# xdu-Liu-learn/Video-desensitization

Hardware: AMD Instinct MI355X
Metric: end-to-end detect+blur FPS on 1920x1080 frames (higher is better)
Workload: dtype fp32; 1 GPU; RetinaFace-R50+FPN+SSH + YOLOv8n plates detect + mosaic write-back, 64 frames of 1920x1080 per step over 1 GPU(s) (batches of 64 per GPU); global_batch=64, frame=1920x1080, net_input=640x640, parallelism=frame-sharded x1, plates=True, batches_in_flight=1

## Files before the change

video-desensitization_amd/csrc/conv_x6.hip:

```cpp
#include "vd_kernel.h"
#include "conv_x6.h"
#include <algorithm>
#include <type_traits>
#include <cmath>
#include <cstring>

namespace {

template <int BM, int BN, int NT, int NST, int TERMS, int MF, bool TR = false, bool PF = false>
__global__ __launch_bounds__(NT, NT == 256 && BM == 256 ? 1 : 2) void conv_x6_kernel(ConvArgs a) {
    static_assert(MF == 16 || (MF == 32 && TERMS == 2), "32x32x16 form: fp16 pairs only");
    static_assert(!TR || (MF == 16 && TERMS == 2), "TR tiles: fp16 pairs on 16x16x32");
    using S = X6Shape<BM, BN, NT, NST, TERMS, MF>;
    constexpr int NA = 2;
    constexpr int STAGE = S::STAGE, PL_A = S::PL_A, PL_B = S::PL_B, TM = S::TM, TN = S::TN, WAVES = S::WAVES;
    constexpr int AROWS = S::AROWS, AIT = S::AITEMS;
    extern __shared__ __attribute__((aligned(16))) char smem[];
    const int tid = threadIdx.x, lane = tid & 63, wid = tid >> 6;
    const int wm = wid / S::WAVES_N, wn = wid % S::WAVES_N;

    const int nwg = gridDim.x, bid = blockIdx.x;
    const int q8 = nwg >> 3, r8 = nwg & 7, xcd = bid & 7;
    const int wg = (xcd < r8 ? xcd * (q8 + 1) : r8 * (q8 + 1) + (xcd - r8) * q8) + (bid >> 3);
    const int tn = wg % a.ntiles_n, tm = wg / a.ntiles_n;
// ... 405 lines not shown
    hipError_t err = hipSuccess;
    if (vd_launch_x6_stream(a, TERMS, s, &err)) return err;
    if constexpr (TERMS == 2) {
        if (a.tune->x6_gemm1x1 && x6_tr_ok(a)) return launch_tr(a, s);
    }
    const int bn = a.cout <= 32 ? 32 : (a.cout <= 64 ? 64 : 128);
    const long big_tiles = (long)((a.M + 255) / 256) * ((a.cout + bn - 1) / bn);
    const int small_k = a.tune->x6_small_k, small_tiles = a.tune->x6_small_tiles, small_k2 = a.tune->x6_small_k2;
    const bool force_small = small_k >= (1 << 30);
    const bool small = force_small || (bn <= 64 && (a.kpad <= (TERMS == 2 ? small_k2 : small_k) ||
                                                    big_tiles < small_tiles));
    if constexpr (TERMS == 2) {
        if (bn <= 64 && a.tune->x6_halo_narrow && vd_x6_halo_ok(a)) return vd_launch_x6_halo(a, bn, s);
    }
    if (small) {
        if constexpr (TERMS == 2) {
            if (bn == 32 && a.x_exact) return launch_x6<128, 32, 256, 1, 1>(a, s);
            if (bn == 64 && a.x_exact) return launch_x6<128, 64, 256, 1, 1>(a, s);
        }
        if (bn == 32) return launch_x6<128, 32, 256, 1, TERMS>(a, s);
        if (bn == 64) return launch_x6<128, 64, 256, 1, TERMS>(a, s);
        return launch_x6<128, 128, 256, 1, TERMS>(a, s);
    }
    if (bn == 32) return launch_x6<256, 32, 512, 2, TERMS>(a, s);
    if (bn == 64) return launch_x6<256, 64, 512, 2, TERMS>(a, s);
    if constexpr (TERMS == 2) {
        if (a.tune->x6_mid && a.kh == 1 && a.kw == 1 && a.kpad <= a.tune->x6_mid && a.cout == 128)
            return launch_x6<128, 128, 256, 2, TERMS>(a, s);
    }
    if constexpr (TERMS == 2) {
        const long t256 = (long)((a.M + 255) / 256) * (a.cout / 256);
        if (a.tune->x6_bn256 && a.cout % 256 == 0 && t256 >= 192) {
            if (vd_x6_halo_ok(a)) return vd_launch_x6_halo(a, 256, s);
            if (a.tune->x6_mf32) return launch_x6<256, 256, 512, 2, TERMS, 32>(a, s);
            return launch_x6<256, 256, 512, 2, TERMS>(a, s);
        }
        if (a.tune->x6_bn256 && a.cout == 192 && (a.M + 255) / 256 >= 192) {
            if (vd_x6_halo_ok(a)) return vd_launch_x6_halo(a, 192, s);
            return launch_x6<256, 192, 512, 2, TERMS>(a, s);
        }
        if (vd_x6_halo_ok(a)) return vd_launch_x6_halo(a, 128, s);
        if (a.tune->x6_mf32) return launch_x6<256, 128, 512, 2, TERMS, 32>(a, s);
    }
    return launch_x6<256, 128, 512, 2, TERMS>(a, s);
}

hipError_t vd_launch_conv_x6(const ConvArgs& a0, hipStream_t s) {
    if (!a0.tune) return hipErrorInvalidValue;
    ConvArgs a = a0;
    a.one = a.tune->x6_one != 0;
    a.halo_dma = a.tune->x6_halo_dma & 3;
    a.gemm_1b = a.tune->x6_gemm_uni == 2;
    a.halo_1b = a.tune->x6_halo_1b != 0;
    a.dbg = a.tune->x6_dbg & 0x3d;
    if (a.grp_co) {
        if (a.grp_co != 64 || a.f32_split != 2 || !a.wx3 || !vd_x6_halo_ok(a) || (a.ymax && a.B > kAmaxFrames))
            return hipErrorInvalidValue;
        a.scale = a.scale_x;
        return vd_launch_x6_halo(a, 64, s);
    }
    if (a.x2) {
        if (!vd_conv1x1_x6_dual_ok(a) || (a.ymax && a.B > kAmaxFrames)) return hipErrorInvalidValue;
        return vd_launch_x6_dual(a, s);
    }
    if (a.f32_split == 2) {
        if (!a.scale_x || (a.ymax && a.B > kAmaxFrames)) return hipErrorInvalidValue;
        return launch_terms<2>(a, s);
    }
    ConvArgs b = a;
    b.xmax = nullptr;
    return launch_terms<3>(b, s);
}

static inline unsigned f2u(float f) { unsigned u; std::memcpy(&u, &f, 4); return u; }
static inline float u2f(unsigned u) { float f; std::memcpy(&f, &u, 4); return f; }

void vd_pack_x6(const float* w, int npad, int kpad, uint16_t* out) {
    const int nk = kpad / KT;
    for (int n = 0; n < npad; ++n)
        for (int t = 0; t < nk; ++t)
            for (int k = 0; k < KT; ++k) {
                const float x = w[(size_t)n * kpad + t * KT + k];
                const unsigned u = f2u(x);
                const float r1 = x - u2f(u & 0xFFFF0000u);
                const unsigned v = f2u(r1);
                const float r2 = r1 - u2f(v & 0xFFFF0000u);
                uint16_t* o = out + (((size_t)n * nk + t) * 3) * KT + k;
                o[0] = (uint16_t)(u >> 16);
                o[KT] = (uint16_t)(v >> 16);
                o[2 * KT] = (uint16_t)(f2u(r2) >> 16);
            }
}

void vd_pack_x3h(const float* w, int npad, int kpad, uint16_t* out, float* row_inv) {
    const int nk = kpad / KT;
    for (int n = 0; n < npad; ++n) {
        float m = 0.f;
        for (int k = 0; k < kpad; ++k) m = std::max(m, std::fabs(w[(size_t)n * kpad + k]));
        int e = 0;
        if (m > 0.f) {
            (void)std::frexp(m, &e);
            e = std::min(100, std::max(-100, 15 - e));
        }
        row_inv[n] = std::ldexp(1.f, -e);
        for (int t = 0; t < nk; ++t)
            for (int k = 0; k < KT; ++k) {
// ... 10 lines not shown
```

video-desensitization_amd/csrc/conv_x6_halo.hip:

```cpp
#include "vd_kernel.h"
#include "conv_x6.h"
#include <algorithm>

namespace {

__device__ __forceinline__ int swzh(int row, int chunk) { return row * 64 + ((chunk ^ (((row >> 2) & 1) << 1)) << 4); }

__host__ __device__ __forceinline__ constexpr int s2_tap(int j) {
    return j == 0 ? 8 : j == 1 ? 6 : j == 2 ? 2 : j == 3 ? 0 : j == 4 ? 7 : j == 5 ? 1 : j == 6 ? 5 : j == 7 ? 3 : 4;
}
__host__ __device__ __forceinline__ constexpr bool s2_last(int j) { return j == 3 || j == 5 || j == 7 || j == 8; }

template <int BN, int NSB, bool TR = false, bool S2 = false, bool PF = false>
__global__ __launch_bounds__(512, BN <= 64 ? 4 : 2) void conv_x6_halo_kernel(ConvArgs a) {
    using S = X6Shape<256, BN, 512, 2, 2>;
    constexpr int BM = 256, NT = 512, TM = S::TM, TN = S::TN, WAVES = S::WAVES, PL_B = S::PL_B;
    constexpr int QI = 4;
    extern __shared__ __attribute__((aligned(16))) char smem[];
    const int tid = threadIdx.x, lane = tid & 63, wid = tid >> 6;
    const int wm = wid / S::WAVES_N, wn = wid % S::WAVES_N;
    const int nwg = gridDim.x, bid = blockIdx.x;
    const int q8 = nwg >> 3, r8 = nwg & 7, xcd = bid & 7;
    const int wg = (xcd < r8 ? xcd * (q8 + 1) : r8 * (q8 + 1) + (xcd - r8) * q8) + (bid >> 3);
    const int tn = wg % a.ntiles_n, tm = wg / a.ntiles_n;
    const int m0 = tm * BM, n0 = tn * BN;
    static_assert(!S2 || (NSB == 3 && S::NDMA % WAVES == 0), "stride-2 halo: three B stages, whole DMA rounds");
    const int W = a.yw, H = a.yh, HW = H * W;
    const int HR = S2 ? BM + W + 1 : BM + 2 * W + 2, HP = HR + 1;
    const int PL_H = HP * 64;
    char* Ah = smem + NSB * 2 * PL_B;
    const int CH = a.cin_pad / 32, nsteps = 9 * CH, nk = a.kpad / KT;
    const int nhalo = S2 ? 4 * CH : CH;

    const long xbytes = (long)a.B * a.xh * a.xw * a.ldx * 4;
    const __amdgpu_buffer_rsrc_t rsrc_x = __builtin_amdgcn_make_buffer_rsrc((void*)a.x, 0, (int)xbytes, 0x00020000);
    int hoff[QI];
    unsigned hexp = 0;
    unsigned hodd = 0;
    const int xg = a.grp_co ? (n0 / a.grp_co) * a.grp_ci : 0;
#pragma unroll
    for (int q = 0; q < QI; ++q) {
        const int it = tid + NT * q, hr = it >> 2, pr = it & 3;
        const int pix = m0 - W - 1 + hr;
        const bool ok = hr < HR && pix >= 0 && pix < a.M;
        if constexpr (S2) {
            const int b = pix / HW, rem = pix - b * HW, yo = rem / W, xo = rem - yo * W;
            hoff[q] = ok ? ((b * a.xh + 2 * yo) * a.xw + 2 * xo) * a.ldx + a.xcoff + xg + pr * 8 : -1;
            hodd |= (unsigned)((2 * yo + 1 < a.xh ? 1 : 0) | (2 * xo + 1 < a.xw ? 2 : 0)) << (2 * q);
        } else {
            hoff[q] = ok ? pix * a.ldx + a.xcoff + xg + pr * 8 : -1;
        }
        hexp |= (unsigned)((ok ? act_scale_exp(a, pix / HW) : 0) & 0xff) << (8 * q);
    }
    u32x4 hx[QI][2];
    auto load_halo = [&](int h) {
        const int c = S2 ? h >> 2 : h, ph = S2 ? 3 - (h & 3) : 0, py = ph >> 1, px = ph & 1;
        const int dph = (py * a.xw + px) * a.ldx;
        const unsigned need = (unsigned)(py | (px << 1));
#pragma unroll
        for (int q = 0; q < QI; ++q) {
            const bool v = hoff[q] >= 0 && (!S2 || ((hodd >> (2 * q)) & need) == need);
            const unsigned off = v ? (unsigned)(hoff[q] + dph + c * KT) * 4u : 0x80000000u;
            hx[q][0] = __builtin_bit_cast(u32x4, __builtin_amdgcn_raw_buffer_load_b128(rsrc_x, (int)off, 0, 0));
            hx[q][1] = __builtin_bit_cast(u32x4, __builtin_amdgcn_raw_buffer_load_b128(rsrc_x, (int)off, 16, 0));
        }
    };
    auto store_halo = [&]() {
#pragma unroll
        for (int q = 0; q < QI; ++q) {
            const int it = tid + NT * q, hr = it >> 2, pr = it & 3;
            if (hr < HR) {
                float e[8];
#pragma unroll
                for (int j = 0; j < 4; ++j) {
                    e[j] = __uint_as_float(hx[q][0][j]);
                    e[4 + j] = __uint_as_float(hx[q][1][j]);
                }
                u32x4 o[3];
                const int ex = (int)(signed char)((hexp >> (8 * q)) & 0xff);
                split_pack<2>(e, __builtin_ldexpf(1.f, ex), o);
                *(u32x4*)(Ah + swzh(hr, pr)) = o[0];
                *(u32x4*)(Ah + PL_H + swzh(hr, pr)) = o[1];
            }
        }
    };

    constexpr int RB = BN / 16, NDMA = S::NDMA;
    const int my_dma = NDMA / WAVES + (wid < NDMA % WAVES ? 1 : 0);
    const __amdgpu_buffer_rsrc_t rsrc_w = __builtin_amdgcn_make_buffer_rsrc((void*)a.w, 0, 0x7fffffff, 0x00020000);
    auto dma_piece = [&](int s, int st, int q) {
        const int c = s / 9, j = s - 9 * c, kt = (S2 ? s2_tap(j) : j) * CH + c;
        char* Bs = smem + st * 2 * PL_B;
        const int jd = wid + WAVES * q;
        if (jd < NDMA) {
            const int p = jd / RB, r0 = (jd % RB) * 16;
            const int row = r0 + (lane >> 2), slot = lane & 3;
            const int chunk = slot ^ (((row >> 3) & 1) * 3);
            const int wrow = TR ? x6_tr_row(row) : row;
            const unsigned off = (unsigned)((((long)(n0 + wrow) * nk + kt) * 2 + p) * 64 + chunk * 16);
            __builtin_amdgcn_raw_ptr_buffer_load_lds(rsrc_w, (lds_void_t*)(Bs + p * PL_B + r0 * 64), 16, off, 0,
                                                     0, 0);
        }
    };
    auto dma_b = [&](int s, int st) {
#pragma unroll
        for (int q = 0; q < (NDMA + WAVES - 1) / WAVES; ++q) dma_piece(s, st, q);
    };
    constexpr int MYD = S::NDMA % WAVES == 0 ? S::NDMA / WAVES : 0;
    const int hdma = MYD ? a.halo_dma & 3 : 0;
    const int hdbg = (a.dbg >> 2) & 15;

    int arow[TM], aflg[TM];
#pragma unroll
    for (int i = 0; i < TM; ++i) {
        const int r = wm * S::WTM + i * 16 + (lane & 15), m = m0 + r;
        const int rem = m % HW, y = rem / W, x = rem - y * W;
        arow[i] = r + W + 1;
        aflg[i] = (y > 0 ? 1 : 0) | (y < H - 1 ? 2 : 0) | (x > 0 ? 4 : 0) | (x < W - 1 ? 8 : 0) | (m < a.M ? 16 : 0);
    }

    using AccT = f32x4_t;
    AccT acc[TM][TN];
#pragma unroll
    for (int i = 0; i < TM; ++i)
#pragma unroll
        for (int j = 0; j < TN; ++j) acc[i][j] = AccT{};
    const int amax_off = std::max(NSB * 2 * PL_B + 2 * PL_H, S::EPR * S::EPLD * 4);
    if (a.ymax)
        for (int f = tid; f < a.B; f += NT) ((unsigned*)(smem + amax_off))[f] = 0u;

    auto compute = [&](int st, int dy, int dx, int dstep) {
        const char* Bs = smem + st * 2 * PL_B;
        const int ch = lane >> 4;
        const int need = S2 ? (dy < 0 ? 1 : 0) | (dx < 0 ? 4 : 0) | 16
                            : (dy < 0 ? 1 : 0) | (dy > 0 ? 2 : 0) | (dx < 0 ? 4 : 0) | (dx > 0 ? 8 : 0) | 16;
        const int shift = S2 ? (dy < 0 ? -W : 0) + (dx < 0 ? -1 : 0) : dy * W + dx;
        if constexpr (TN < TM) {
            u32x4 bf[TN][3];
#pragma unroll
            for (int j = 0; j < TN; ++j) {
                bf[j][0] = *(const u32x4*)(Bs + swz64(wn * S::WTN + j * 16 + (lane & 15), ch));
                bf[j][1] = *(const u32x4*)(Bs + PL_B + swz64(wn * S::WTN + j * 16 + (lane & 15), ch));
            }
#pragma unroll
            for (int i = 0; i < TM; ++i) {
                const int hr = (aflg[i] & need) == need ? arow[i] + shift : HR;
                const int o = swzh(hr, ch);
                u32x4 af[3];
                af[0] = *(const u32x4*)(Ah + o);
                af[1] = *(const u32x4*)(Ah + PL_H + o);
#pragma unroll
                for (int j = 0; j < TN; ++j) {
                    if constexpr (TR) acc[i][j] = mfma_pair_tr(af, bf[j], acc[i][j]);
                    else acc[i][j] = mfma_pair(af, bf[j], acc[i][j]);
                }
            }
        } else if constexpr (PF) {
            u32x4 af[TM][3], bq[2][3];
#pragma unroll
            for (int i = 0; i < TM; ++i) {
                const int hr = (aflg[i] & need) == need ? arow[i] + shift : HR;
                const int o = swzh(hr, ch);
                af[i][0] = *(const u32x4*)(Ah + o);
                af[i][1] = *(const u32x4*)(Ah + PL_H + o);
            }
            bq[0][0] = *(const u32x4*)(Bs + swz64(wn * S::WTN + (lane & 15), ch));
            bq[0][1] = *(const u32x4*)(Bs + PL_B + swz64(wn * S::WTN + (lane & 15), ch));
            __builtin_amdgcn_sched_group_barrier(0x0100, 2 * TM + 2, 0);
#pragma unroll
            for (int j = 0; j < TN; ++j) {
                if (j + 1 < TN) {
                    bq[(j + 1) & 1][0] = *(const u32x4*)(Bs + swz64(wn * S::WTN + (j + 1) * 16 + (lane & 15), ch));
                    bq[(j + 1) & 1][1] = *(const u32x4*)(Bs + PL_B + swz64(wn * S::WTN + (j + 1) * 16 + (lane & 15), ch));
                    __builtin_amdgcn_sched_group_barrier(0x0100, 2, 0);
                }
#pragma unroll
                for (int i = 0; i < TM; ++i) {
                    if constexpr (TR) acc[i][j] = mfma_pair_tr(af[i], bq[j & 1], acc[i][j]);
                    else acc[i][j] = mfma_pair(af[i], bq[j & 1], acc[i][j]);
                }
                __builtin_amdgcn_sched_group_barrier(0x0008, 3 * TM, 0);
                if constexpr (MYD > 0 && TN % MYD == 0) {
                    if (dstep >= 0 && j % (TN / MYD) == 0) dma_piece(dstep, dstep % NSB, j / (TN / MYD));
                }
            }
        } else {
            u32x4 af[TM][3];
#pragma unroll
            for (int i = 0; i < TM; ++i) {
                const int hr = (aflg[i] & need) == need ? arow[i] + shift : HR;
                const int o = swzh(hr, ch);
                af[i][0] = *(const u32x4*)(Ah + o);
                af[i][1] = *(const u32x4*)(Ah + PL_H + o);
            }
#pragma unroll
            for (int j = 0; j < TN; ++j) {
                u32x4 bf[3];
                bf[0] = *(const u32x4*)(Bs + swz64(wn * S::WTN + j * 16 + (lane & 15), ch));
                bf[1] = *(const u32x4*)(Bs + PL_B + swz64(wn * S::WTN + j * 16 + (lane & 15), ch));
#pragma unroll
                for (int i = 0; i < TM; ++i) {
                    if constexpr (TR) acc[i][j] = mfma_pair_tr(af[i], bf, acc[i][j]);
                    else acc[i][j] = mfma_pair(af[i], bf, acc[i][j]);
                }
                if constexpr (MYD > 0 && TN % MYD == 0) {
                    if (dstep >= 0 && j % (TN / MYD) == 0) dma_piece(dstep, dstep % NSB, j / (TN / MYD));
                }
            }
        }
    };

    load_halo(0);
    store_halo();
    if (tid < 8) *(u32x4*)(Ah + (tid >> 2) * PL_H + swzh(HR, tid & 3)) = u32x4{0u, 0u, 0u, 0u};
    dma_b(0, 0);
    const bool one_bar = NSB == 2 && MYD > 0 && a.halo_1b;
    if (nsteps > 1 && !one_bar) dma_b(1, 1);
    if (nhalo > 1) load_halo(1);
    if constexpr (NSB == 3 && S::NDMA % WAVES == 0) {
        int hcur = 0;
        for (int s = 0; s < nsteps; ++s) {
            const int tap = s % 9;
            const bool ended = s >= 1 && (S2 ? s2_last(tap == 0 ? 8 : tap - 1) : tap == 0);
            const bool halo_prev = ended ? hcur + 1 < nhalo : (s <= 1 && nhalo > 1);
            if (halo_prev) {
                if (s + 1 < nsteps) wait_vm_k<MYD + 2 * QI>();
                else wait_vm_k<2 * QI>();
            } else {
                if (s + 1 < nsteps) wait_vm_k<MYD>();
                else wait_vm_k<0>();
            }
            asm volatile("s_waitcnt lgkmcnt(0)" ::: "memory");
            if (!(hdbg & 8)) __builtin_amdgcn_s_barrier();
            asm volatile("" ::: "memory");
            const bool rehalo = (S2 ? s2_last(tap) : tap == 8) && hcur + 1 < nhalo;
            const bool dnext = !rehalo && s + 2 < nsteps && !(hdbg & 1);
            const int hd = (TN % (MYD ? MYD : 1) == 0 && TN >= TM) ? hdma : (hdma ? 1 : 0);
            if (dnext && hd == 0) dma_b(s + 2, (s + 2) % 3);
            const int wt = S2 ? s2_tap(tap) : tap;
            const int dy = wt / 3 - 1, dx = wt - (wt / 3) * 3 - 1;
            compute(s % 3, dy, dx, dnext && hd == 2 ? s + 2 : -1);
            if (dnext && hd == 1) dma_b(s + 2, (s + 2) % 3);
            if (rehalo) {
                asm volatile("s_waitcnt lgkmcnt(0)" ::: "memory");
                if (!(hdbg & 8)) __builtin_amdgcn_s_barrier();
                asm volatile("" ::: "memory");
                if (!(hdbg & 2)) store_halo();
                ++hcur;
                if (hcur + 1 < nhalo && !(hdbg & 2)) load_halo(hcur + 1);
                if (s + 2 < nsteps && !(hdbg & 1)) dma_b(s + 2, (s + 2) % 3);
            }
        }
    } else if constexpr (NSB == 3) {
        for (int s = 0; s < nsteps; ++s) {
            const int c = s / 9, tap = s - 9 * c;
            const bool halo_prev = (s >= 1 && (s - 1) % 9 == 8 && (s - 1) / 9 + 2 < CH) || (s <= 1 && CH > 1);
            const int younger = (s + 1 < nsteps ? my_dma : 0) + (halo_prev ? 2 * QI : 0);
            wait_vm(younger);
            asm volatile("s_waitcnt lgkmcnt(0)" ::: "memory");
            __builtin_amdgcn_s_barrier();
            asm volatile("" ::: "memory");
            const bool rehalo = tap == 8 && c + 1 < CH;
            if (!rehalo && s + 2 < nsteps) dma_b(s + 2, (s + 2) % 3);
            const int dy = tap / 3 - 1, dx = tap - (tap / 3) * 3 - 1;
            compute(s % 3, dy, dx, -1);
            if (rehalo) {
                asm volatile("s_waitcnt lgkmcnt(0)" ::: "memory");
                __builtin_amdgcn_s_barrier();
                asm volatile("" ::: "memory");
                store_halo();
                if (c + 2 < CH) load_halo(c + 2);
                if (s + 2 < nsteps) dma_b(s + 2, (s + 2) % 3);
            }
        }
    } else if (one_bar) {
        int hcur = 0;
        for (int s = 0; s < nsteps; ++s) {
            const int tap = s % 9;
            const bool halo_prev = s == 0 ? nhalo > 1 : (tap == 0 && hcur + 1 < nhalo);
            if (halo_prev) wait_vm_k<2 * QI>();
            else wait_vm_k<0>();
            asm volatile("s_waitcnt lgkmcnt(0)" ::: "memory");
            if (!(hdbg & 8)) __builtin_amdgcn_s_barrier();
            asm volatile("" ::: "memory");
            if (s + 1 < nsteps && !(hdbg & 1)) dma_b(s + 1, (s + 1) & 1);
            const int dy = tap / 3 - 1, dx = tap - (tap / 3) * 3 - 1;
            compute(s & 1, dy, dx, -1);
            if (tap == 8 && hcur + 1 < nhalo) {
                asm volatile("s_waitcnt lgkmcnt(0)" ::: "memory");
                if (!(hdbg & 8)) __builtin_amdgcn_s_barrier();
                asm volatile("" ::: "memory");
                if (!(hdbg & 2)) store_halo();
                ++hcur;
                if (hcur + 1 < nhalo && !(hdbg & 2)) load_halo(hcur + 1);
            }
        }
    } else {
    for (int s = 0; s < nsteps; ++s) {
        const int c = s / 9, tap = s - 9 * c;
        int younger = s + 1 < nsteps ? my_dma : 0;
        if (s == 0 && CH > 1) younger += 2 * QI;
        if (s == 1 && CH > 1) younger = 2 * QI + (s + 1 < nsteps ? my_dma : 0);
        if (s >= 2 && tap == 0 && c + 1 < CH) younger += 2 * QI;
        wait_vm(younger);
        asm volatile("s_waitcnt lgkmcnt(0)" ::: "memory");
        __builtin_amdgcn_s_barrier();
        asm volatile("" ::: "memory");
        const int dy = tap / 3 - 1, dx = tap - (tap / 3) * 3 - 1;
        compute(s & 1, dy, dx, -1);
        asm volatile("s_waitcnt lgkmcnt(0)" ::: "memory");
        __builtin_amdgcn_s_barrier();
        asm volatile("" ::: "memory");
        if (tap == 8 && c + 1 < CH) {
            store_halo();
            if (c + 2 < CH) load_halo(c + 2);
        }
        if (s + 2 < nsteps) dma_b(s + 2, s & 1);
    }
    }
    if constexpr (TR) {
        x6_epilogue_tr<S>(a, acc, m0, n0, wm, wn, lane, (unsigned*)(smem + amax_off));
    } else {
        __syncthreads();
        x6_epilogue<S, 16>(a, acc, m0, n0, wm, wn, tid, lane, smem, amax_off);
    }
}

template <int BN, int NSB>
static int x6_halo_lds(const ConvArgs& a) {
    using S = X6Shape<256, BN, 512, 2, 2>;
    const int HP = a.stride == 2 ? 256 + a.yw + 2 : 256 + 2 * a.yw + 3;
    return std::max(NSB * 2 * S::PL_B + 2 * HP * 64, S::EPR * S::EPLD * 4) + (a.ymax ? 4 * a.B : 0);
}

template <int BN, int NSB, bool TR, bool S2, bool PF>
static hipError_t launch_x6_halo_pf(const ConvArgs& a0, hipStream_t s) {
    ConvArgs a = a0;
    a.w = a.wx3;
    a.ntiles_n = (a.cout + BN - 1) / BN;
    static const bool attr = [] {
        (void)hipFuncSetAttribute((const void*)conv_x6_halo_kernel<BN, NSB, TR, S2, PF>,
                                  hipFuncAttributeMaxDynamicSharedMemorySize, 160 * 1024);
        return true;
    }();
    (void)attr;
    const int lds = x6_halo_lds<BN, NSB>(a);
    if (lds > 160 * 1024) return hipErrorInvalidValue;
    const int mt = (a.M + 255) / 256;
    hipLaunchKernelGGL((conv_x6_halo_kernel<BN, NSB, TR, S2, PF>), dim3(mt * a.ntiles_n), dim3(512), lds, s, a);
    return hipGetLastError();
}

template <int BN, int NSB, bool TR = false, bool S2 = false>
static hipError_t launch_x6_halo_t(const ConvArgs& a, hipStream_t s) {
    if constexpr (BN >= 128) {
        if (a.tune->x6_halo_pf) return launch_x6_halo_pf<BN, NSB, TR, S2, true>(a, s);
    }
    return launch_x6_halo_pf<BN, NSB, TR, S2, false>(a, s);
}

template <int BN, int NSB>
static hipError_t launch_x6_halo_n(const ConvArgs& a, hipStream_t s) {
    const bool tr = a.tune->x6_halo_tr >= (BN >= 128 ? 1 : 2) && !((a.ldy | a.ycoff) & 7) && tr_bytes_ok(a) &&
                    (a.res_mode == VD_RES_NONE || !((a.res_ld | a.res_coff) & 7));
    if constexpr (NSB == 3 && BN >= 64) {
        if (a.stride == 2) return tr ? launch_x6_halo_t<BN, 3, true, true>(a, s) : launch_x6_halo_t<BN, 3, false, true>(a, s);
    }
    if (a.stride != 1) return hipErrorInvalidValue;
    if (tr) return launch_x6_halo_t<BN, NSB, true>(a, s);
    return launch_x6_halo_t<BN, NSB, false>(a, s);
}

template <int BN>
static hipError_t launch_x6_halo(const ConvArgs& a, hipStream_t s) {
    if ((a.tune->x6_halo >= 2 || a.stride == 2) && x6_halo_lds<BN, 3>(a) <= 160 * 1024) return launch_x6_halo_n<BN, 3>(a, s);
    return launch_x6_halo_n<BN, 2>(a, s);
}

}

bool vd_x6_halo_ok(const ConvArgs& a) {
    if (!a.tune->x6_halo || a.kh != 3 || a.kw != 3 || a.pad != 1) return false;
    if (a.cin_pad % 32 || a.kpad != 9 * a.cin_pad || (a.ymax && a.B > kAmaxFrames)) return false;
    if (a.stride == 2) {
        if (!a.tune->x6_halo_s2 || a.cout <= 32 || a.grp_co) return false;
        if (a.yh != (a.xh - 1) / 2 + 1 || a.yw != (a.xw - 1) / 2 + 1 || 256 + a.yw + 2 > 512) return false;
        return (3 * 2 * 256 * 64 + 2 * (256 + a.yw + 2) * 64 + (a.ymax ? 4 * a.B : 0)) <= 160 * 1024;
    }
    if (a.stride != 1 || a.xh != a.yh || a.xw != a.yw) return false;
    if (256 + 2 * a.yw + 2 > 512) return false;
    return true;
}

hipError_t vd_launch_x6_halo(const ConvArgs& a, int bn, hipStream_t s) {
    if (bn == 32) return launch_x6_halo<32>(a, s);
    if (bn == 64) return launch_x6_halo<64>(a, s);
    if (bn == 128) return launch_x6_halo<128>(a, s);
    if (bn == 192) return launch_x6_halo<192>(a, s);
    if (bn == 256) return launch_x6_halo<256>(a, s);
    return hipErrorInvalidValue;
}
```

video-desensitization_amd/csrc/runtime.cpp:

```cpp
#include "../../include/vdmi.h"
#include "vd_common.h"
#include "vd_math.h"
#include "nets.h"

#include <algorithm>
#include <cmath>
#include <cstdarg>
#include <cstdio>
#include <cstdlib>
#include <cstring>
#include <mutex>
#include <string>
#include <thread>
#include <vector>

static thread_local std::string g_err;

static bool vd_ranges_overlap(const void* a, const void* b, size_t bytes) {
    const uintptr_t x = (uintptr_t)a, y = (uintptr_t)b;
    return bytes && x < y + bytes && y < x + bytes;
}

int vd_set_error(int code, const char* fmt, ...) {
    char buf[1024];
// ... 1112 lines not shown

int vd_load_weights(vd_ctx* h, int net, const void* blob, size_t bytes, int fmt) {
    Ctx* ctx = (Ctx*)h;
    VD_ENTRY(ctx);
    if (fmt != VD_WEIGHTS_VDW1) return vd_set_error(VD_ERR_ARG, "unknown weight format %d", fmt);
    if (!blob) return vd_set_error(VD_ERR_ARG, "null weight blob");
    WMap W;
    int rc = vd_parse_vdw1(blob, bytes, W);
    if (rc) return rc;
    if (net == VD_NET_RETINAFACE) {
        if (ctx->face.loaded) return vd_set_error(VD_ERR_STATE, "RetinaFace weights already loaded");
        return vd_build_face(*ctx, W);
    }
    if (net == VD_NET_YOLOV8N) {
        if (ctx->plate.loaded) return vd_set_error(VD_ERR_STATE, "plate weights already loaded");
        return vd_build_plate(*ctx, W);
    }
    return vd_set_error(VD_ERR_ARG, "unknown net %d", net);
}

int vd_set_option(vd_ctx* h, const char* name, int value) {
    Ctx* ctx = (Ctx*)h;
    VD_ENTRY(ctx);
    if (!name) return vd_set_error(VD_ERR_ARG, "null option name");
    struct Opt { const char* n; int VdTune::*f; };
    static const Opt opts[] = {
        {"conv_stream", &VdTune::conv_stream}, {"conv_stream512", &VdTune::conv_stream512},
        {"conv_dual", &VdTune::conv_dual}, {"conv_taps", &VdTune::conv_taps}, {"conv_n192", &VdTune::conv_n192},
        {"conv_small", &VdTune::conv_small}, {"conv_big", &VdTune::conv_big},
        {"conv_big_kmin", &VdTune::conv_big_kmin}, {"stream_ntt", &VdTune::stream_ntt},
        {"lb_pair", &VdTune::lb_pair}, {"mosaic_map", &VdTune::mosaic_map}, {"mosaic_nt", &VdTune::mosaic_nt},
        {"mosaic_cells", &VdTune::mosaic_cells}, {"mosaic_fused", &VdTune::mosaic_fused},
        {"mosaic_rows", &VdTune::mosaic_rows}, {"mosaic_gather", &VdTune::mosaic_gather},
        {"block_fuse", &VdTune::block_fuse}, {"block_fuse32", &VdTune::block_fuse32},
        {"block32_xd", &VdTune::block32_xd}, {"block32_pipe", &VdTune::block32_pipe}, {"chain", &VdTune::chain},
        {"chain_gpw", &VdTune::chain_gpw}, {"stem_pool", &VdTune::stem_pool}, {"ssh_fuse", &VdTune::ssh_fuse},
        {"ssh_side", &VdTune::ssh_side},
        {"plate_s2d", &VdTune::plate_s2d}, {"plate_s2d32", &VdTune::plate_s2d32},
        {"plate_stage", &VdTune::plate_stage}, {"plate_detect_early", &VdTune::plate_detect_early},
        {"mosaic_early", &VdTune::mosaic_early}, {"face_groups", &VdTune::face_groups},
        {"det_group", &VdTune::det_group}, {"f32_split", &VdTune::f32_split},
        {"x6_small_k", &VdTune::x6_small_k}, {"x6_small_k2", &VdTune::x6_small_k2},
        {"x6_small_tiles", &VdTune::x6_small_tiles}, {"x6_bn256", &VdTune::x6_bn256},
        {"x6_exact", &VdTune::x6_exact}, {"x6_mid", &VdTune::x6_mid}, {"x6_mf32", &VdTune::x6_mf32},
        {"x6_one", &VdTune::x6_one},
        {"x6_stream", &VdTune::x6_stream}, {"x6_stream_silu", &VdTune::x6_stream_silu},
        {"x6_stream_rl", &VdTune::x6_stream_rl}, {"x6_stream256", &VdTune::x6_stream256},
        {"x6_taps", &VdTune::x6_taps},
        {"x6_gemm1x1", &VdTune::x6_gemm1x1}, {"x6_gemm_uni", &VdTune::x6_gemm_uni},
        {"x6_gemm_pf", &VdTune::x6_gemm_pf},
        {"x6_halo", &VdTune::x6_halo}, {"x6_halo_narrow", &VdTune::x6_halo_narrow},
        {"x6_halo_s2", &VdTune::x6_halo_s2}, {"x6_halo_tr", &VdTune::x6_halo_tr},
        {"x6_halo_dma", &VdTune::x6_halo_dma}, {"x6_halo_pf", &VdTune::x6_halo_pf},
        {"x6_halo_1b", &VdTune::x6_halo_1b},
        {"jenc_gpu", &VdTune::jenc_gpu}, {"jdec_gpu", &VdTune::jdec_gpu}, {"jdec_chunk", &VdTune::jdec_chunk},
        {"jdec_sync", &VdTune::jdec_sync}, {"jdec_group", &VdTune::jdec_group},
    };
    for (const Opt& o : opts)
        if (strcmp(o.n, name) == 0) {
            if (!strcmp(name, "stream_ntt") && value != 8 && value != 16)
                return vd_set_error(VD_ERR_ARG, "stream_ntt must be 8 or 16");
            if (!strcmp(name, "x6_gemm_uni") && value != 0 && value != 2)
                return vd_set_error(VD_ERR_ARG, "x6_gemm_uni must be 0 or 2");
            ctx->tune.*(o.f) = value;
            return VD_OK;
        }
    return vd_set_error(VD_ERR_ARG, "unknown option '%s'", name);
}

int vdt_set_debug(vd_ctx* h, const char* name, int value) {
    Ctx* ctx = (Ctx*)h;
    VD_ENTRY(ctx);
    if (!name) return vd_set_error(VD_ERR_ARG, "null debug switch name");
    if (!strcmp(name, "x6_dbg")) { ctx->tune.x6_dbg = value; return VD_OK; }
    if (!strcmp(name, "block32_dbg")) { ctx->tune.block32_dbg = value; return VD_OK; }
    return vd_set_error(VD_ERR_ARG, "unknown debug switch '%s'", name);
}

int vd_set_stream(vd_ctx* h, void* s) {
    Ctx* ctx = (Ctx*)h;
    VD_ENTRY(ctx);
    ctx->stream = s ? (hipStream_t)s : ctx->own_stream;
    return VD_OK;
}

void* vd_get_stream(vd_ctx* h) { return h ? (void*)((Ctx*)h)->stream : nullptr; }

int vd_sync(vd_ctx* h) {
    Ctx* ctx = (Ctx*)h;
    VD_ENTRY(ctx);
    VD_CHECK_HIP(hipStreamSynchronize(ctx->stream));
    return VD_OK;
}

int vd_detect(vd_ctx* h, const uint8_t* frames, int n, int fh, int fw, size_t pitch, int where, vd_boxes* faces) {
    Ctx* ctx = (Ctx*)h;
    VD_ENTRY(ctx);
    if (!ctx->face.loaded) return vd_set_error(VD_ERR_STATE, "RetinaFace weights not loaded");
    int rc = ctx->check_frames(n, fh, fw, pitch);
    if (rc) return rc;
    BoxTargets t;
    rc = ctx->box_targets(faces, n, t);
    if (rc) return rc;
    const uint8_t* d = ctx->frames_to_device(frames, n, fh, pitch, where, &rc);
    if (rc) return rc;
    if ((rc = ctx->face_letterbox(d, n, fh, fw, pitch))) return rc;
    if ((rc = ctx->face_forward(n))) return rc;
// ... 576 lines not shown
```

video-desensitization_amd/csrc/vd_common.h:

```cpp
#pragma once
#include <hip/hip_runtime.h>
#include <hip/hip_bf16.h>
#include <stdint.h>
#include <stddef.h>

enum VdAct { VD_ACT_NONE = 0, VD_ACT_RELU = 1, VD_ACT_LEAKY = 2, VD_ACT_SILU = 3 };
enum VdResMode { VD_RES_NONE = 0, VD_RES_PRE_ACT = 1, VD_RES_POST_ACT = 2 };

struct VdTune {
    int conv_stream = 1;
    int conv_stream512 = 1;
    int conv_dual = 1;
    int conv_taps = 1;
    int conv_n192 = 1;
    int conv_small = 512;
    int conv_big = 100;
    int conv_big_kmin = 512;
    int stream_ntt = 16;
    int lb_pair = 1;
    int mosaic_map = 1;
    int mosaic_nt = 0;
    int mosaic_cells = 32;
    int mosaic_gather = 0;
    int mosaic_rows = 0;
    int mosaic_fused = 1;
    int block_fuse = 1;
    int block32_xd = 2;
    int block32_dbg = 0;
    int block32_pipe = 1;
    int block_fuse32 = 1;
    int chain = 2;
    int stem_pool = 1;
    int ssh_fuse = 2;
    int plate_s2d = 1;
    int jenc_gpu = 1;
    int jdec_gpu = 1;
    int jdec_sync = 128;
    int jdec_chunk = 1024;
    int jdec_group = 4;
    int ssh_side = 0;
    int chain_gpw = 1;
    int det_group = 1;
    int plate_s2d32 = 1;
    int face_groups = 2;
    int plate_detect_early = 1;
    int mosaic_early = 1;
    int plate_stage = 3;
    int x6_stream = 1;
    int x6_stream_rl = 1;
    int x6_stream_silu = 1;
    int x6_stream256 = 2;
    int x6_small_k = 256;
    int x6_small_tiles = 512;
    int x6_small_k2 = 1 << 20;
    int x6_bn256 = 1;
    int x6_exact = 1;
    int x6_mid = 512;
    int x6_mf32 = 0;
    int x6_halo = 2;
    int x6_halo_narrow = 1;
    int x6_halo_s2 = 1;
    int x6_halo_1b = 1;
    int x6_gemm_uni = 2;
    int x6_gemm_pf = 1;
    int x6_halo_pf = 1;
    int x6_halo_dma = 2;
    int x6_halo_tr = 2;
    int x6_one = 1;
    int x6_taps = 1;
    int x6_gemm1x1 = 1;
    int x6_dbg = 0;
    int f32_split = 2;
};

struct ConvArgs {
    const void* x;  int xh, xw, ldx, xcoff;
    const void* w;
    const float* scale; const float* shift;
    const void* res; int res_ld, res_coff, res_up;
    int rh, rw;
    void* y;  int yh, yw, ldy, ycoff;
    int B, cin_pad, cout, kpad;
    int kh, kw, stride, pad;
    int M;
    int act; float slope; int res_mode; int out_f32;
    int f16;
    int ntiles_n;
    const void* x2; int xh2, xw2, ldx2, xcoff2, stride2;
    const void* w2; const float* scale2; const float* shift2; int cin2_pad, kpad2;
    const VdTune* tune;
    const void* wx3;
    const float* scale_x;
    int f32_split;
    const unsigned* xmax; float xbound;
    unsigned* ymax;
    const void* wx3_2; const float* scale2_x;
    const unsigned* x2max; float x2bound;
    int x_exact;
    int one;
    int halo_dma;
    int gemm_1b;
    int halo_1b;
    int dbg;
    int grp_co, grp_ci;
};

struct BlockArgs {
    const void* x; void* y;
    int B, H, W, cin, ds;
    int tiles_x, tiles_y;
    const void* w1;
    const void* w2;
    const void* w3;
    const void* wd;
    const float* bn;
    unsigned long long* diag;
    int mode;
    int f16;
};

struct Block32Args {
    const void* x; void* y;
    int B, H, W, cin, ds;
    int tiles_x, tiles_y;
    const void* w1;
    const void* w2;
    const void* w3;
    const void* wd;
    const float* bn;
    const unsigned* xmax;
    unsigned* ymax;
    int xdepth;
    int pipe;
    int dbg;
};

struct ChainArgs {
    const void* t2; int ld_t2;
    const void* res; int ld_res;
    const void* w3; int kpad3;
    const float* sc3; const float* sh3;
    const void* w1; int kpad1;
    const float* sc1; const float* sh1;
    void* y; int ld_y;
    void* y2; int ld_y2;
    int M;
    int f16;
};

struct Chain32Args {
    const void* t2; int ld_t2;
    const void* res; int ld_res;
    const void* w3;
    const void* w1;
    const float* sc3; const float* sh3;
    const float* sc1; const float* sh1;
    void* y; int ld_y;
// ... 228 lines not shown
```

Before: 2813 frames/s.

## Double-buffer halo tiles in x6 halo conv to overlap halo staging with MFMA

Adds a ping-pong (two-set) halo buffer variant of the 3x3 halo conv kernel for BN=128 with three B stages, enabled by default via a new x6_halo_pp tune flag. The next channel chunk's halo is written into the alternate LDS set while the current set is read, and on stride-2 some store steps interleave halo stores and loads with the MFMA columns under scheduling barriers. This removes the extra barrier and exposed halo store at each chunk boundary. The cost is double the halo LDS footprint, which may lower occupancy or fall back when LDS exceeds 160KB, plus more intricate wait-count logic.

Measured after the change: 2802 frames/s. No clear change (-0.4%).

```diff
diff --git a/video-desensitization_amd/csrc/conv_x6.hip b/video-desensitization_amd/csrc/conv_x6.hip
--- a/video-desensitization_amd/csrc/conv_x6.hip
+++ b/video-desensitization_amd/csrc/conv_x6.hip
@@ -481,6 +481,7 @@
     a.halo_dma = a.tune->x6_halo_dma & 3;
     a.gemm_1b = a.tune->x6_gemm_uni == 2;
     a.halo_1b = a.tune->x6_halo_1b != 0;
+    a.halo_pp = a.tune->x6_halo_pp != 0;
     a.dbg = a.tune->x6_dbg & 0x3d;
     if (a.grp_co) {
         if (a.grp_co != 64 || a.f32_split != 2 || !a.wx3 || !vd_x6_halo_ok(a) || (a.ymax && a.B > kAmaxFrames))
diff --git a/video-desensitization_amd/csrc/conv_x6_halo.hip b/video-desensitization_amd/csrc/conv_x6_halo.hip
--- a/video-desensitization_amd/csrc/conv_x6_halo.hip
+++ b/video-desensitization_amd/csrc/conv_x6_halo.hip
@@ -1,6 +1,7 @@
 #include "vd_kernel.h"
 #include "conv_x6.h"
 #include <algorithm>
+#include <type_traits>
 
 namespace {
 
@@ -10,8 +11,10 @@
     return j == 0 ? 8 : j == 1 ? 6 : j == 2 ? 2 : j == 3 ? 0 : j == 4 ? 7 : j == 5 ? 1 : j == 6 ? 5 : j == 7 ? 3 : 4;
 }
 __host__ __device__ __forceinline__ constexpr bool s2_last(int j) { return j == 3 || j == 5 || j == 7 || j == 8; }
-
-template <int BN, int NSB, bool TR = false, bool S2 = false, bool PF = false>
+__host__ __device__ __forceinline__ constexpr bool s2_store(int j) { return j == 1 || j == 4 || j == 6 || j == 8; }
+constexpr int kS1Store = 4;
+
+template <int BN, int NSB, bool TR = false, bool S2 = false, bool PF = false, bool PP = false>
 __global__ __launch_bounds__(512, BN <= 64 ? 4 : 2) void conv_x6_halo_kernel(ConvArgs a) {
     using S = X6Shape<256, BN, 512, 2, 2>;
     constexpr int BM = 256, NT = 512, TM = S::TM, TN = S::TN, WAVES = S::WAVES, PL_B = S::PL_B;
@@ -25,10 +28,12 @@
     const int tn = wg % a.ntiles_n, tm = wg / a.ntiles_n;
     const int m0 = tm * BM, n0 = tn * BN;
     static_assert(!S2 || (NSB == 3 && S::NDMA % WAVES == 0), "stride-2 halo: three B stages, whole DMA rounds");
+    static_assert(!PP || (NSB == 3 && S::NDMA % WAVES == 0), "two halo sets: three B stages, whole DMA rounds");
     const int W = a.yw, H = a.yh, HW = H * W;
     const int HR = S2 ? BM + W + 1 : BM + 2 * W + 2, HP = HR + 1;
     const int PL_H = HP * 64;
     char* Ah = smem + NSB * 2 * PL_B;
+    const char* Ar = Ah;
     const int CH = a.cin_pad / 32, nsteps = 9 * CH, nk = a.kpad / KT;
     const int nhalo = S2 ? 4 * CH : CH;
 
@@ -65,7 +70,7 @@
             hx[q][1] = __builtin_bit_cast(u32x4, __builtin_amdgcn_raw_buffer_load_b128(rsrc_x, (int)off, 16, 0));
         }
     };
-    auto store_halo = [&]() {
+    auto store_halo = [&](char* Ad) {
 #pragma unroll
         for (int q = 0; q < QI; ++q) {
             const int it = tid + NT * q, hr = it >> 2, pr = it & 3;
@@ -79,11 +84,36 @@
                 u32x4 o[3];
                 const int ex = (int)(signed char)((hexp >> (8 * q)) & 0xff);
                 split_pack<2>(e, __builtin_ldexpf(1.f, ex), o);
-                *(u32x4*)(Ah + swzh(hr, pr)) = o[0];
-                *(u32x4*)(Ah + PL_H + swzh(hr, pr)) = o[1];
-            }
-        }
-    };
+                *(u32x4*)(Ad + swzh(hr, pr)) = o[0];
+                *(u32x4*)(Ad + PL_H + swzh(hr, pr)) = o[1];
+            }
+        }
+    };
+    auto store_item = [&](char* Ad, int q) {
+        const int it = tid + NT * q, hr = std::min(it >> 2, HR), pr = it & 3;
+        float e[8];
+#pragma unroll
+        for (int j = 0; j < 4; ++j) {
+            e[j] = __uint_as_float(hx[q][0][j]);
+            e[4 + j] = __uint_as_float(hx[q][1][j]);
+        }
+        u32x4 o[3];
+        const int ex = (int)(signed char)((hexp >> (8 * q)) & 0xff);
+        split_pack<2>(e, __builtin_ldexpf(1.f, ex), o);
+        *(u32x4*)(Ad + swzh(hr, pr)) = o[0];
+        *(u32x4*)(Ad + PL_H + swzh(hr, pr)) = o[1];
+    };
+    auto load_item = [&](int h, int q) {
+        const int c = S2 ? h >> 2 : h, ph = S2 ? 3 - (h & 3) : 0, py = ph >> 1, px = ph & 1;
+        const int dph = (py * a.xw + px) * a.ldx;
+        const unsigned need = (unsigned)(py | (px << 1));
+        const bool v = h < nhalo && hoff[q] >= 0 && (!S2 || ((hodd >> (2 * q)) & need) == need);
+        const unsigned off = v ? (unsigned)(hoff[q] + dph + c * KT) * 4u : 0x80000000u;
+        hx[q][0] = __builtin_bit_cast(u32x4, __builtin_amdgcn_raw_buffer_load_b128(rsrc_x, (int)off, 0, 0));
+        hx[q][1] = __builtin_bit_cast(u32x4, __builtin_amdgcn_raw_buffer_load_b128(rsrc_x, (int)off, 16, 0));
+    };
+    char* Aw = Ah;
+    int hnext = 0;
 
     constexpr int RB = BN / 16, NDMA = S::NDMA;
     const int my_dma = NDMA / WAVES + (wid < NDMA % WAVES ? 1 : 0);
@@ -125,11 +155,13 @@
     for (int i = 0; i < TM; ++i)
 #pragma unroll
         for (int j = 0; j < TN; ++j) acc[i][j] = AccT{};
-    const int amax_off = std::max(NSB * 2 * PL_B + 2 * PL_H, S::EPR * S::EPLD * 4);
+    const int amax_off = std::max(NSB * 2 * PL_B + (PP ? 4 : 2) * PL_H, S::EPR * S::EPLD * 4);
     if (a.ymax)
         for (int f = tid; f < a.B; f += NT) ((unsigned*)(smem + amax_off))[f] = 0u;
 
-    auto compute = [&](int st, int dy, int dx, int dstep) {
+    auto compute_t = [&](auto SI, int st, int dy, int dx, int dstep) {
+        constexpr bool SIV = decltype(SI)::value;
+        static_assert(!SIV || (PP && TN >= TM && TN == QI), "a store step pairs the halo items with the column blocks");
         const char* Bs = smem + st * 2 * PL_B;
         const int ch = lane >> 4;
         const int need = S2 ? (dy < 0 ? 1 : 0) | (dx < 0 ? 4 : 0) | 16
@@ -147,8 +179,8 @@
                 const int hr = (aflg[i] & need) == need ? arow[i] + shift : HR;
                 const int o = swzh(hr, ch);
                 u32x4 af[3];
-                af[0] = *(const u32x4*)(Ah + o);
-                af[1] = *(const u32x4*)(Ah + PL_H + o);
+                af[0] = *(const u32x4*)(Ar + o);
+                af[1] = *(const u32x4*)(Ar + PL_H + o);
 #pragma unroll
                 for (int j = 0; j < TN; ++j) {
                     if constexpr (TR) acc[i][j] = mfma_pair_tr(af, bf[j], acc[i][j]);
@@ -161,8 +193,8 @@
             for (int i = 0; i < TM; ++i) {
                 const int hr = (aflg[i] & need) == need ? arow[i] + shift : HR;
                 const int o = swzh(hr, ch);
-                af[i][0] = *(const u32x4*)(Ah + o);
-                af[i][1] = *(const u32x4*)(Ah + PL_H + o);
+                af[i][0] = *(const u32x4*)(Ar + o);
+                af[i][1] = *(const u32x4*)(Ar + PL_H + o);
             }
             bq[0][0] = *(const u32x4*)(Bs + swz64(wn * S::WTN + (lane & 15), ch));
             bq[0][1] = *(const u32x4*)(Bs + PL_B + swz64(wn * S::WTN + (lane & 15), ch));
@@ -179,10 +211,22 @@
                     if constexpr (TR) acc[i][j] = mfma_pair_tr(af[i], bq[j & 1], acc[i][j]);
                     else acc[i][j] = mfma_pair(af[i], bq[j & 1], acc[i][j]);
                 }
+                if constexpr (SIV) {
+                    store_item(Aw, j);
+                    load_item(hnext, j);
+#pragma unroll
+                    for (int g = 0; g < 3 * TM; ++g) {
+                        __builtin_amdgcn_sched_group_barrier(0x0008, 1, 0);
+                        __builtin_amdgcn_sched_group_barrier(0x0002, 3, 0);
+                    }
+                    __builtin_amdgcn_sched_group_barrier(0x0200, 2, 0);
+                    __builtin_amdgcn_sched_group_barrier(0x0020, 2, 0);
+                } else {
                 __builtin_amdgcn_sched_group_barrier(0x0008, 3 * TM, 0);
                 if constexpr (MYD > 0 && TN % MYD == 0) {
                     if (dstep >= 0 && j % (TN / MYD) == 0) dma_piece(dstep, dstep % NSB, j / (TN / MYD));
                 }
+                }
             }
         } else {
             u32x4 af[TM][3];
@@ -190,8 +234,8 @@
             for (int i = 0; i < TM; ++i) {
                 const int hr = (aflg[i] & need) == need ? arow[i] + shift : HR;
                 const int o = swzh(hr, ch);
-                af[i][0] = *(const u32x4*)(Ah + o);
-                af[i][1] = *(const u32x4*)(Ah + PL_H + o);
+                af[i][0] = *(const u32x4*)(Ar + o);
+                af[i][1] = *(const u32x4*)(Ar + PL_H + o);
             }
 #pragma unroll
             for (int j = 0; j < TN; ++j) {
@@ -203,21 +247,113 @@
                     if constexpr (TR) acc[i][j] = mfma_pair_tr(af[i], bf, acc[i][j]);
                     else acc[i][j] = mfma_pair(af[i], bf, acc[i][j]);
                 }
-                if constexpr (MYD > 0 && TN % MYD == 0) {
+                if constexpr (SIV) {
+                    store_item(Aw, j);
+                    load_item(hnext, j);
+                } else if constexpr (MYD > 0 && TN % MYD == 0) {
                     if (dstep >= 0 && j % (TN / MYD) == 0) dma_piece(dstep, dstep % NSB, j / (TN / MYD));
                 }
             }
         }
     };
 
+    auto compute = [&](int st, int dy, int dx, int dstep) { compute_t(std::false_type{}, st, dy, dx, dstep); };
+
     load_halo(0);
-    store_halo();
-    if (tid < 8) *(u32x4*)(Ah + (tid >> 2) * PL_H + swzh(HR, tid & 3)) = u32x4{0u, 0u, 0u, 0u};
+    store_halo(Ah);
+    if (tid < (PP ? 16 : 8)) *(u32x4*)(Ah + (tid >> 2) * PL_H + swzh(HR, tid & 3)) = u32x4{0u, 0u, 0u, 0u};
+    if constexpr (PP) {
+        if (nhalo > 1) load_halo(1);
+        asm volatile("" ::: "memory");
+        __builtin_amdgcn_sched_barrier(0);
+    }
     dma_b(0, 0);
     const bool one_bar = NSB == 2 && MYD > 0 && a.halo_1b;
     if (nsteps > 1 && !one_bar) dma_b(1, 1);
-    if (nhalo > 1) load_halo(1);
-    if constexpr (NSB == 3 && S::NDMA % WAVES == 0) {
+    if (!PP && nhalo > 1) load_halo(1);
+    if constexpr (PP) {
+        int hcur = 0, hl = -3;
+        if constexpr (S2) {
+            for (int s = 0; s < nsteps; ++s) {
+                const int tap = s % 9;
+                if (s - hl <= 1) {
+                    if (s + 1 < nsteps) wait_vm_k<MYD + 2 * QI>();
+                    else wait_vm_k<2 * QI>();
+                } else {
+                    if (s + 1 < nsteps) wait_vm_k<MYD>();
+                    else wait_vm_k<0>();
+                }
+                asm volatile("s_waitcnt lgkmcnt(0)" ::: "memory");
+                __builtin_amdgcn_s_barrier();
+                asm volatile("" ::: "memory");
+                const bool sstep = s2_store(tap) && hcur + 1 < nhalo;
+                const bool dnext = s + 2 < nsteps;
+                const int hd = sstep ? 1 : (TN % (MYD ? MYD : 1) == 0 && TN >= TM) ? hdma : (hdma ? 1 : 0);
+                if (dnext && hd == 0) dma_b(s + 2, (s + 2) % 3);
+                const int wt = s2_tap(tap);
+                const int dy = wt / 3 - 1, dx = wt - (wt / 3) * 3 - 1;
+                if (sstep) {
+                    Aw = Ah + ((hcur + 1) & 1) * 2 * PL_H;
+                    hnext = hcur + 2;
+                    hl = s;
+                    asm volatile("" ::: "memory");
+                    __builtin_amdgcn_sched_barrier(0);
+                    compute_t(std::true_type{}, s % 3, dy, dx, -1);
+                    asm volatile("" ::: "memory");
+                    __builtin_amdgcn_sched_barrier(0);
+                } else {
+                    compute(s % 3, dy, dx, dnext && hd == 2 ? s + 2 : -1);
+                }
+                if (dnext && hd == 1) dma_b(s + 2, (s + 2) % 3);
+                if (s2_last(tap)) {
+                    ++hcur;
+                    Ar = Ah + (hcur & 1) * 2 * PL_H;
+                }
+            }
+        } else {
+            for (int s = 0; s < nsteps; ++s) {
+                const int tap = s % 9;
+                if (s - hl <= 2) {
+                    if (s + 1 < nsteps) wait_vm_k<MYD + 2 * QI>();
+                    else wait_vm_k<2 * QI>();
+                } else {
+                    if (s + 1 < nsteps) wait_vm_k<MYD>();
+                    else wait_vm_k<0>();
+                }
+                asm volatile("s_waitcnt lgkmcnt(0)" ::: "memory");
+                __builtin_amdgcn_s_barrier();
+                asm volatile("" ::: "memory");
+                const bool sstep = tap == kS1Store && hcur + 1 < nhalo;
+                const bool dnext = s + 2 < nsteps;
+                const int hd = (TN % (MYD ? MYD : 1) == 0 && TN >= TM) ? hdma : (hdma ? 1 : 0);
+                if (!sstep && dnext && hd == 0) dma_b(s + 2, (s + 2) % 3);
+                const int dy = tap / 3 - 1, dx = tap - (tap / 3) * 3 - 1;
+                if (sstep) Aw = Ah + ((hcur + 1) & 1) * 2 * PL_H;
+                compute(s % 3, dy, dx, !sstep && dnext && hd == 2 ? s + 2 : -1);
+                if (!sstep && dnext && hd == 1) dma_b(s + 2, (s + 2) % 3);
+                if (sstep) {
+                    __builtin_amdgcn_sched_barrier(0);
+                    wait_vm_k<MYD>();
+                    store_halo(Aw);
+                    asm volatile("" ::: "memory");
+                    __builtin_amdgcn_sched_barrier(0);
+                    if (dnext) dma_b(s + 2, (s + 2) % 3);
+                    asm volatile("" ::: "memory");
+                    __builtin_amdgcn_sched_barrier(0);
+                    if (hcur + 2 < nhalo) {
+                        load_halo(hcur + 2);
+                        hl = s;
+                    }
+                    asm volatile("" ::: "memory");
+                    __builtin_amdgcn_sched_barrier(0);
+                }
+                if (tap == 8) {
+                    ++hcur;
+                    Ar = Ah + (hcur & 1) * 2 * PL_H;
+                }
+            }
+        }
+    } else if constexpr (NSB == 3 && S::NDMA % WAVES == 0) {
         int hcur = 0;
         for (int s = 0; s < nsteps; ++s) {
             const int tap = s % 9;
@@ -245,7 +381,7 @@
                 asm volatile("s_waitcnt lgkmcnt(0)" ::: "memory");
                 if (!(hdbg & 8)) __builtin_amdgcn_s_barrier();
                 asm volatile("" ::: "memory");
-                if (!(hdbg & 2)) store_halo();
+                if (!(hdbg & 2)) store_halo(Ah);
                 ++hcur;
                 if (hcur + 1 < nhalo && !(hdbg & 2)) load_halo(hcur + 1);
                 if (s + 2 < nsteps && !(hdbg & 1)) dma_b(s + 2, (s + 2) % 3);
@@ -268,7 +404,7 @@
                 asm volatile("s_waitcnt lgkmcnt(0)" ::: "memory");
                 __builtin_amdgcn_s_barrier();
                 asm volatile("" ::: "memory");
-                store_halo();
+                store_halo(Ah);
                 if (c + 2 < CH) load_halo(c + 2);
                 if (s + 2 < nsteps) dma_b(s + 2, (s + 2) % 3);
             }
@@ -290,7 +426,7 @@
                 asm volatile("s_waitcnt lgkmcnt(0)" ::: "memory");
                 if (!(hdbg & 8)) __builtin_amdgcn_s_barrier();
                 asm volatile("" ::: "memory");
-                if (!(hdbg & 2)) store_halo();
+                if (!(hdbg & 2)) store_halo(Ah);
                 ++hcur;
                 if (hcur + 1 < nhalo && !(hdbg & 2)) load_halo(hcur + 1);
             }
@@ -312,7 +448,7 @@
         __builtin_amdgcn_s_barrier();
         asm volatile("" ::: "memory");
         if (tap == 8 && c + 1 < CH) {
-            store_halo();
+            store_halo(Ah);
             if (c + 2 < CH) load_halo(c + 2);
         }
         if (s + 2 < nsteps) dma_b(s + 2, s & 1);
@@ -326,33 +462,40 @@
     }
 }
 
-template <int BN, int NSB>
-static int x6_halo_lds(const ConvArgs& a) {
+static int x6_halo_lds(int bn, int nsb, int sets, const ConvArgs& a) {
+    const int HP = a.stride == 2 ? 256 + a.yw + 2 : 256 + 2 * a.yw + 3;
+    return std::max(nsb * 2 * bn * 64 + sets * 2 * HP * 64, 128 * (bn + 4) * 4) + (a.ymax ? 4 * a.B : 0);
+}
+constexpr int kHaloLdsMax = 160 * 1024;
+
+template <int BN, int NSB, bool TR, bool S2, bool PF, bool PP = false>
+static hipError_t launch_x6_halo_pf(const ConvArgs& a0, hipStream_t s) {
     using S = X6Shape<256, BN, 512, 2, 2>;
-    const int HP = a.stride == 2 ? 256 + a.yw + 2 : 256 + 2 * a.yw + 3;
-    return std::max(NSB * 2 * S::PL_B + 2 * HP * 64, S::EPR * S::EPLD * 4) + (a.ymax ? 4 * a.B : 0);
-}
-
-template <int BN, int NSB, bool TR, bool S2, bool PF>
-static hipError_t launch_x6_halo_pf(const ConvArgs& a0, hipStream_t s) {
+    static_assert(S::PL_B == BN * 64 && S::EPR == 128 && S::EPLD == BN + 4, "x6_halo_lds restates these");
     ConvArgs a = a0;
     a.w = a.wx3;
     a.ntiles_n = (a.cout + BN - 1) / BN;
     static const bool attr = [] {
-        (void)hipFuncSetAttribute((const void*)conv_x6_halo_kernel<BN, NSB, TR, S2, PF>,
-                                  hipFuncAttributeMaxDynamicSharedMemorySize, 160 * 1024);
+        (void)hipFuncSetAttribute((const void*)conv_x6_halo_kernel<BN, NSB, TR, S2, PF, PP>,
+                                  hipFuncAttributeMaxDynamicSharedMemorySize, kHaloLdsMax);
         return true;
     }();
     (void)attr;
-    const int lds = x6_halo_lds<BN, NSB>(a);
-    if (lds > 160 * 1024) return hipErrorInvalidValue;
+    const int lds = x6_halo_lds(BN, NSB, PP ? 2 : 1, a);
+    if (lds > kHaloLdsMax) return hipErrorInvalidValue;
     const int mt = (a.M + 255) / 256;
-    hipLaunchKernelGGL((conv_x6_halo_kernel<BN, NSB, TR, S2, PF>), dim3(mt * a.ntiles_n), dim3(512), lds, s, a);
+    hipLaunchKernelGGL((conv_x6_halo_kernel<BN, NSB, TR, S2, PF, PP>), dim3(mt * a.ntiles_n), dim3(512), lds, s, a);
     return hipGetLastError();
 }
 
 template <int BN, int NSB, bool TR = false, bool S2 = false>
 static hipError_t launch_x6_halo_t(const ConvArgs& a, hipStream_t s) {
+    if constexpr (BN == 128 && NSB == 3) {
+        if (a.halo_pp && x6_halo_lds(BN, 3, 2, a) <= kHaloLdsMax) {
+            if (a.tune->x6_halo_pf) return launch_x6_halo_pf<BN, NSB, TR, S2, true, true>(a, s);
+            return launch_x6_halo_pf<BN, NSB, TR, S2, false, true>(a, s);
+        }
+    }
     if constexpr (BN >= 128) {
         if (a.tune->x6_halo_pf) return launch_x6_halo_pf<BN, NSB, TR, S2, true>(a, s);
     }
@@ -373,7 +516,7 @@
 
 template <int BN>
 static hipError_t launch_x6_halo(const ConvArgs& a, hipStream_t s) {
-    if ((a.tune->x6_halo >= 2 || a.stride == 2) && x6_halo_lds<BN, 3>(a) <= 160 * 1024) return launch_x6_halo_n<BN, 3>(a, s);
+    if ((a.tune->x6_halo >= 2 || a.stride == 2) && x6_halo_lds(BN, 3, 1, a) <= kHaloLdsMax) return launch_x6_halo_n<BN, 3>(a, s);
     return launch_x6_halo_n<BN, 2>(a, s);
 }
 
@@ -385,7 +528,7 @@
     if (a.stride == 2) {
         if (!a.tune->x6_halo_s2 || a.cout <= 32 || a.grp_co) return false;
         if (a.yh != (a.xh - 1) / 2 + 1 || a.yw != (a.xw - 1) / 2 + 1 || 256 + a.yw + 2 > 512) return false;
-        return (3 * 2 * 256 * 64 + 2 * (256 + a.yw + 2) * 64 + (a.ymax ? 4 * a.B : 0)) <= 160 * 1024;
+        return x6_halo_lds(256, 3, 1, a) <= kHaloLdsMax;
     }
     if (a.stride != 1 || a.xh != a.yh || a.xw != a.yw) return false;
     if (256 + 2 * a.yw + 2 > 512) return false;
diff --git a/video-desensitization_amd/csrc/runtime.cpp b/video-desensitization_amd/csrc/runtime.cpp
--- a/video-desensitization_amd/csrc/runtime.cpp
+++ b/video-desensitization_amd/csrc/runtime.cpp
@@ -1188,7 +1188,7 @@
         {"x6_halo", &VdTune::x6_halo}, {"x6_halo_narrow", &VdTune::x6_halo_narrow},
         {"x6_halo_s2", &VdTune::x6_halo_s2}, {"x6_halo_tr", &VdTune::x6_halo_tr},
         {"x6_halo_dma", &VdTune::x6_halo_dma}, {"x6_halo_pf", &VdTune::x6_halo_pf},
-        {"x6_halo_1b", &VdTune::x6_halo_1b},
+        {"x6_halo_1b", &VdTune::x6_halo_1b}, {"x6_halo_pp", &VdTune::x6_halo_pp},
         {"jenc_gpu", &VdTune::jenc_gpu}, {"jdec_gpu", &VdTune::jdec_gpu}, {"jdec_chunk", &VdTune::jdec_chunk},
         {"jdec_sync", &VdTune::jdec_sync}, {"jdec_group", &VdTune::jdec_group},
     };
diff --git a/video-desensitization_amd/csrc/vd_common.h b/video-desensitization_amd/csrc/vd_common.h
--- a/video-desensitization_amd/csrc/vd_common.h
+++ b/video-desensitization_amd/csrc/vd_common.h
@@ -61,6 +61,7 @@
     int x6_halo_narrow = 1;
     int x6_halo_s2 = 1;
     int x6_halo_1b = 1;
+    int x6_halo_pp = 1;
     int x6_gemm_uni = 2;
     int x6_gemm_pf = 1;
     int x6_halo_pf = 1;
@@ -103,6 +104,7 @@
     int halo_1b;
     int dbg;
     int grp_co, grp_ci;
+    int halo_pp;
 };
 
 struct BlockArgs {
```
